# genjax-community/genjax

Hardware: AMD Instinct MI355X
Metric: particle_steps_per_sec (higher is better)
Workload: dtype f32; 1 GPU; gmm_c8_d16 ImportanceK: propagate+reweight+LSE, systematic resample, gather (BASELINE.json configs[1]); k_particles_per_gpu=1048576, k_particles_total=1048576, rng_stream=flat, exchange=none

## Files before the change

### genjax_amd/csrc/gjx_resample.hip

```cpp
#include <math.h>
#include <string.h>

#include "gjx_device.h"
#include "gjx_host.h"
#include "gjx_scan.h"
#include "gjx_tile.h"

namespace gjx {

struct PickPair {
  float v;
  int32_t i;
};

GJX_DEV void pick_better(float& v, int32_t& i, float ov, int32_t oi) {
  if (ov > v || (ov == v && oi < i)) { v = ov; i = oi; }
}

template <int RNG>
__global__ __launch_bounds__(256) void k_pick_partial(const float* logw, int64_t K, int64_t offset, const float* lse,
                                                     key2 key, PickPair* partials) {
  __shared__ float rv[4];
  __shared__ int32_t ri[4];
  const float l = lse[2];
// ... 115 lines not shown
  const int64_t base = (int64_t)blockIdx.x * kScanTile + (int64_t)threadIdx.x * kScanItems;
  uint64_t s = 0;
#pragma unroll
  for (int k = 0; k < kScanItems; ++k)
    if (base + k < K) s += weight_q(x, base + k, is_log, mx);
  s = wave_sum_u64(s);
  if ((threadIdx.x & 63) == 0) red[threadIdx.x >> 6] = s;
  __syncthreads();
  if (threadIdx.x == 0) block_sums[blockIdx.x] = red[0] + red[1] + red[2] + red[3];
}

__global__ __launch_bounds__(256) void k_wscan_write(const float* x, int64_t K, int is_log, const float* lse,
                                                    int n_partials, const uint64_t* block_sums, uint64_t* cum,
                                                    uint64_t* base_total) {
  __shared__ uint64_t wsum[4];
  __shared__ uint64_t red[4];
  __shared__ float fred[8];
  const float mx = block_ref_max(is_log, lse, n_partials, fred, nullptr);
  const int64_t base = (int64_t)blockIdx.x * kScanTile + (int64_t)threadIdx.x * kScanItems;
  uint64_t pre = 0;
  for (int t = threadIdx.x; t < (int)blockIdx.x; t += 256) pre += block_sums[t];
  pre = wave_sum_u64(pre);
  if ((threadIdx.x & 63) == 0) red[threadIdx.x >> 6] = pre;
  uint64_t q[kScanItems];
  uint64_t s = 0;
#pragma unroll
  for (int k = 0; k < kScanItems; ++k) {
    q[k] = (base + k < K) ? weight_q(x, base + k, is_log, mx) : 0;
    s += q[k];
    q[k] = s;
  }
  uint64_t inc = wave_scan_u64(s);
  if ((threadIdx.x & 63) == 63) wsum[threadIdx.x >> 6] = inc;
  __syncthreads();
  uint64_t off = red[0] + red[1] + red[2] + red[3] + inc - s;
  for (int w = 0; w < (int)(threadIdx.x >> 6); ++w) off += wsum[w];
#pragma unroll
  for (int k = 0; k < kScanItems; ++k)
    if (base + k < K) cum[base + k] = off + q[k];
  if (blockIdx.x == gridDim.x - 1 && threadIdx.x == 255) {
    base_total[0] = 0;
    base_total[1] = off + s;
  }
}

GJX_DEV int64_t upper_search(const uint64_t* __restrict__ cum, int64_t K, uint64_t t) {
  int64_t lo = 0, hi = K - 1;
  while (lo < hi) {
    const int64_t mid = (lo + hi) >> 1;
    if (cum[mid] > t) hi = mid; else lo = mid + 1;
  }
  return lo;
}

GJX_DEV int64_t upper_search_in(const uint64_t* __restrict__ cum, int64_t lo, int64_t hi, uint64_t t) {
  while (lo < hi) {
    const int64_t mid = (lo + hi) >> 1;
    if (cum[mid] > t) hi = mid; else lo = mid + 1;
  }
  return lo;
}

template <bool GATHER>
__global__ __launch_bounds__(256) void k_systematic_expand(const uint64_t* __restrict__ cum, int64_t K,
                                                          const uint64_t* base_total, double u, int64_t N_total,
                                                          int64_t out_begin, int64_t n_out, int32_t* ancestors,
                                                          const float* __restrict__ src, int64_t src_stride, int rows,
                                                          float* __restrict__ dst, int64_t dst_stride,
                                                          const int64_t* range_dev = nullptr) {
  constexpr int kOwn = 8;
  if (range_dev) {
    out_begin = range_dev[0];
    const int64_t n = range_dev[1];
    n_out = n < n_out ? n : n_out;
  }
  __shared__ int n_heavy;
  __shared__ int32_t h_i[256];
  __shared__ int64_t h_lo[256], h_hi[256];
  if (threadIdx.x == 0) n_heavy = 0;
  __syncthreads();
  const int64_t i = (int64_t)blockIdx.x * 256 + threadIdx.x;
  const uint64_t base = base_total[0], total = base_total[1];
  const double step = (double)total / (double)N_total;
  const double inv_step = (double)N_total / (double)total;
  const bool in = i < K && total > 0;
  const uint64_t c_cur = in ? base + cum[i] : 0;
  const int64_t j_cur = in ? slots_below(c_cur, u, step, inv_step, total, N_total) : 0;
  int64_t j_prev = __shfl_up((long long)j_cur, 1, 64);
  uint64_t c_prev = __shfl_up((unsigned long long)c_cur, 1, 64);
  if ((threadIdx.x & 63) == 0) {
    c_prev = base + ((in && i > 0) ? cum[i - 1] : 0);
    j_prev = in ? slots_below(c_prev, u, step, inv_step, total, N_total) : 0;
  }
  if (in) {
    if (c_cur > c_prev) {
      int64_t lo = j_prev - out_begin;
      int64_t hi = j_cur - out_begin;
      lo = lo < 0 ? 0 : lo;
      hi = hi > n_out ? n_out : hi;
      if (hi - lo > kOwn) {
        const int h = atomicAdd(&n_heavy, 1);
        h_i[h] = (int32_t)i; h_lo[h] = lo; h_hi[h] = hi;
      } else if (hi > lo) {
        if (ancestors) for (int64_t j = lo; j < hi; ++j) ancestors[j] = (int32_t)i;
        if (GATHER) {
          for (int r = 0; r < rows; ++r) {
            const float v = src[(int64_t)r * src_stride + i];
            for (int64_t j = lo; j < hi; ++j) dst[(int64_t)r * dst_stride + j] = v;
          }
        }
      }
    }
  }
  __syncthreads();
  const int nh = n_heavy;
  for (int h = 0; h < nh; ++h) {
    const int32_t pi = h_i[h];
    const int64_t lo = h_lo[h], hi = h_hi[h];
    if (ancestors) for (int64_t j = lo + threadIdx.x; j < hi; j += 256) ancestors[j] = pi;
    if (GATHER) {
      for (int r = 0; r < rows; ++r) {
        const float v = src[(int64_t)r * src_stride + pi];
        for (int64_t j = lo + threadIdx.x; j < hi; j += 256) dst[(int64_t)r * dst_stride + j] = v;
      }
    }
  }
}

template <int ITEMS>
__global__ __launch_bounds__(256) void k_resample_fused(const float* __restrict__ x, int64_t K, int mode,
                                                       const float* lse, int n_partials, float* lse_out,
                                                       float log_k_total, double u, int64_t N, int32_t* ancestors,
                                                       uint64_t* cum_out, uint64_t* base_total_out,
                                                       unsigned long long* agg, unsigned* ctrl) {
  __shared__ float fred[8];
  __shared__ ScanSmem sm;
  unsigned epoch;
  const unsigned long long tag = grid_tag(ctrl, &epoch);
  const int64_t i0 = ((int64_t)blockIdx.x * 256 + threadIdx.x) * ITEMS;
  float xv[ITEMS];
#pragma unroll
  for (int k = 0; k < ITEMS; ++k) xv[k] = (i0 + k < K) ? x[i0 + k] : 0.0f;
  float sm_sum;
  const float mx = block_ref_max(mode, lse, n_partials, fred, &sm_sum);
  if (mode == 2 && lse_out && blockIdx.x == 0 && threadIdx.x == 0) {
    const float l = mx > -INFINITY ? mx + logf(sm_sum) : -INFINITY;
    lse_out[0] = mx; lse_out[1] = sm_sum; lse_out[2] = l; lse_out[3] = l - log_k_total;
  }
  tile_scan_expand<ITEMS, false>(xv, mode, mx, i0, K, u, N, ancestors, cum_out, base_total_out, agg, tag, ctrl, epoch, true, sm);
}

constexpr int kGatherMaxTiles = 1024;

template <int ITEMS>
__global__ __launch_bounds__(256) void k_resample_gather(const float* __restrict__ x, int64_t K, int mode,
                                                        const float* lse, int n_partials, float* lse_out,
                                                        float log_k_total, double u, const float* __restrict__ src,
                                                        int64_t src_stride, int rows, float* __restrict__ dst,
                                                        int64_t dst_stride, int32_t* ancestors,
                                                        unsigned long long* agg, unsigned* ctrl,
                                                        unsigned long long* timeline) {
#define GJX_STAMP(n) do { if (timeline && threadIdx.x == 0) timeline[blockIdx.x * 8 + (n)] = __builtin_amdgcn_s_memrealtime(); } while (0)
  GJX_STAMP(0);
  constexpr int TILE = 256 * ITEMS;
  __shared__ float fred[8];
  __shared__ uint64_t wsum[4];
  __shared__ uint64_t P[kGatherMaxTiles + 1];
  constexpr int CH = 3;
  __shared__ uint64_t cumL[CH * TILE];
  __shared__ uint64_t s_wtot[CH][4];
  __shared__ int s_range[2];
  unsigned epoch;
  const unsigned long long tag = grid_tag(ctrl, &epoch);
  const int nb = (int)gridDim.x;
  const int lane = threadIdx.x & 63, wid = threadIdx.x >> 6;
  const int64_t i0 = ((int64_t)blockIdx.x * 256 + threadIdx.x) * ITEMS;
  auto load_tile = [&](int64_t p0, float (&v)[ITEMS]) {
    if (ITEMS == 4 && p0 + 4 <= K) {
      const float4 q4 = *(const float4*)(x + p0);
      v[0] = q4.x; v[1] = q4.y; v[2] = q4.z; v[3] = q4.w;
    } else {
#pragma unroll
      for (int k = 0; k < ITEMS; ++k) v[k] = (p0 + k < K) ? x[p0 + k] : 0.0f;
    }
  };
  const int w0 = (int)blockIdx.x - 1;
  float xv[ITEMS], xn[2][ITEMS];
  load_tile(i0, xv);
  float sm_sum;
  const float mx = block_ref_max(mode, lse, n_partials, fred, &sm_sum);
  if (mode == 2 && lse_out && blockIdx.x == 0 && threadIdx.x == 0) {
    const float l = mx > -INFINITY ? mx + logf(sm_sum) : -INFINITY;
    lse_out[0] = mx; lse_out[1] = sm_sum; lse_out[2] = l; lse_out[3] = l - log_k_total;
  }
  uint64_t qown[ITEMS], sown = 0, incown;
  {
#pragma unroll
    for (int k = 0; k < ITEMS; ++k) { sown += (i0 + k < K) ? weight_q(xv, k, mode, mx) : 0; qown[k] = sown; }
    incown = wave_scan_u64(sown);
    if (lane == 63) { wsum[wid] = incown; s_wtot[1][wid] = incown; }
    __syncthreads();
    if (threadIdx.x == 0) grid_publish(agg, tag, wsum[0] + wsum[1] + wsum[2] + wsum[3]);
  }
  GJX_STAMP(1);
#pragma unroll
  for (int c = 0; c < 2; ++c) {
    const int tc = w0 + 2 * c;
#pragma unroll
    for (int k = 0; k < ITEMS; ++k) xn[c][k] = 0.0f;
    if (tc >= 0 && tc < nb) load_tile((int64_t)tc * TILE + (int64_t)threadIdx.x * ITEMS, xn[c]);
  }
  {
    uint64_t qn[2][ITEMS], sn[2], incn[2];
#pragma unroll
    for (int c = 0; c < 2; ++c) {
      const int tc = w0 + 2 * c;
      const bool on = tc >= 0 && tc < nb;
      const int64_t p0 = (int64_t)tc * TILE + (int64_t)threadIdx.x * ITEMS;
      sn[c] = 0;
#pragma unroll
      for (int k = 0; k < ITEMS; ++k) { sn[c] += (on && p0 + k < K) ? weight_q(xn[c], k, mode, mx) : 0; qn[c][k] = sn[c]; }
    }
#pragma unroll
    for (int c = 0; c < 2; ++c) incn[c] = wave_scan_u64(sn[c]);
    if (lane == 63) { s_wtot[0][wid] = incn[0]; s_wtot[2][wid] = incn[1]; }
    __syncthreads();
#pragma unroll
    for (int c = 0; c < 3; ++c) {
      uint64_t base = c == 1 ? incown - sown : incn[c >> 1] - sn[c >> 1];
      for (int w = 0; w < wid; ++w) base += s_wtot[c][w];
#pragma unroll
      for (int k = 0; k < ITEMS; ++k) cumL[c * TILE + threadIdx.x * ITEMS + k] = base + (c == 1 ? qown[k] : qn[c >> 1][k]);
    }
  }
  grid_gather(agg, tag, ctrl, [&](int b, unsigned long long val) { P[b + 1] = val; });
  if (threadIdx.x == 0) P[0] = 0;
  __syncthreads();
  GJX_STAMP(2);
  {
    const int per = (nb + 255) >> 8;
    const int e0 = threadIdx.x * per, e1 = (e0 + per) < nb ? (e0 + per) : nb;
    uint64_t loc = 0;
    for (int e = e0; e < e1; ++e) loc += P[e + 1];
    uint64_t inc = wave_scan_u64(loc);
    if (lane == 63) wsum[wid] = inc;
    __syncthreads();
    uint64_t run = inc - loc;
    for (int w = 0; w < wid; ++w) run += wsum[w];
    for (int e = e0; e < e1; ++e) { run += P[e + 1]; P[e + 1] = run; }
    __syncthreads();
  }
  const uint64_t total = P[nb];
  GJX_STAMP(6);
  if (blockIdx.x == 0 && threadIdx.x == 0) {
    __hip_atomic_store(&ctrl[0], epoch + 1u, __ATOMIC_RELAXED, __HIP_MEMORY_SCOPE_AGENT);
    if (total == 0) __hip_atomic_fetch_or(&ctrl[2], kStatusZeroTotal, __ATOMIC_RELAXED, __HIP_MEMORY_SCOPE_AGENT);
  }
  int32_t anc[ITEMS];
#pragma unroll
  for (int k = 0; k < ITEMS; ++k) anc[k] = (int32_t)((i0 + k < K) ? i0 + k : 0);
  if (total > 0) {
    const double step = (double)total / (double)K;
    uint64_t T[ITEMS];
    int tile[ITEMS], kpos[ITEMS];
#pragma unroll
    for (int k = 0; k < ITEMS; ++k) {
      const int64_t j = (i0 + k < K) ? i0 + k : K - 1;
      T[k] = comb_threshold(j, u, step, total);
      tile[k] = 0;
    }
    auto descend = [&](int k0, int k1) {
#pragma unroll
      for (int sft = kGatherMaxTiles >> 1; sft >= 1; sft >>= 1) {
        const int pa = tile[k0] + sft, pb = tile[k1] + sft;
        if (pa <= nb - 1 && P[pa] <= T[k0]) tile[k0] = pa;
        if (k1 != k0 && pb <= nb - 1 && P[pb] <= T[k1]) tile[k1] = pb;
      }
    };
    const int wlo = (int)blockIdx.x - 4 < 0 ? 0 : ((int)blockIdx.x - 4 > nb - 8 ? (nb - 8 < 0 ? 0 : nb - 8) : (int)blockIdx.x - 4);
    uint64_t Pw[9];
#pragma unroll
    for (int k = 0; k < 9; ++k) Pw[k] = P[wlo + k < nb ? wlo + k : nb];
    if (T[0] >= Pw[0] && T[ITEMS - 1] < Pw[8]) {
#pragma unroll
      for (int k = 0; k < ITEMS; ++k) {
        int tl = wlo;
#pragma unroll
        for (int w = 1; w < 8; ++w) tl += Pw[w] <= T[k] ? 1 : 0;
        tile[k] = tl;
      }
    } else {
      descend(0, ITEMS - 1);
      if (ITEMS > 2) {
        if (tile[0] == tile[ITEMS - 1]) {
#pragma unroll
          for (int k = 1; k < ITEMS - 1; ++k) tile[k] = tile[0];
        } else {
          descend(1, ITEMS > 3 ? 2 : 1);
        }
      }
    }
    if (timeline) { asm volatile("" :: "v"(tile[0]), "v"(tile[ITEMS - 1])); GJX_STAMP(7); }
    if (threadIdx.x == 0) s_range[0] = tile[0];
    if (threadIdx.x == 255) s_range[1] = tile[ITEMS - 1];
    __syncthreads();
    const int tmin = s_range[0], ntiles = s_range[1] - tmin + 1;
    if (tmin >= w0 && s_range[1] <= w0 + 2) {
      GJX_STAMP(3);
      int pos[ITEMS];
      const uint64_t* cm[ITEMS];
      uint64_t Tr[ITEMS];
#pragma unroll
      for (int k = 0; k < ITEMS; ++k) { cm[k] = cumL + (tile[k] - w0) * TILE; Tr[k] = T[k] - P[tile[k]]; pos[k] = 0; }
#pragma unroll
      for (int q = TILE >> 2; q >= 1; q >>= 2) {
#pragma unroll
        for (int k = 0; k < ITEMS; ++k) {
          const uint64_t pa = cm[k][pos[k] + q - 1], pb = cm[k][pos[k] + 2 * q - 1], pc = cm[k][pos[k] + 3 * q - 1];
          pos[k] += (pa <= Tr[k] ? q : 0) + (pb <= Tr[k] ? q : 0) + (pc <= Tr[k] ? q : 0);
        }
      }
#pragma unroll
      for (int k = 0; k < ITEMS; ++k) anc[k] = (int32_t)((int64_t)tile[k] * TILE + pos[k]);
    } else {
#pragma unroll
    for (int k = 0; k < ITEMS; ++k) kpos[k] = tile[k] - tmin;
    auto next_live = [&](int at) { while (at < ntiles && P[tmin + at + 1] == P[tmin + at]) ++at; return at; };
    GJX_STAMP(3);
    float nv[CH][ITEMS];
#pragma unroll
    for (int c = 0; c < CH; ++c)
      if (c < ntiles) load_tile((int64_t)(tmin + c) * TILE + (int64_t)threadIdx.x * ITEMS, nv[c]);
    for (int idx = 0; idx < ntiles;) {
      const int nidx = next_live(idx + CH);
      uint64_t qi[CH][ITEMS], sacc[CH], inc[CH];
      int tsrc[CH];
#pragma unroll
      for (int c = 0; c < CH; ++c) {
        const bool on = idx + c < ntiles;
        tsrc[c] = on ? tmin + idx + c : 0;
        const int64_t p0 = (int64_t)tsrc[c] * TILE + (int64_t)threadIdx.x * ITEMS;
        sacc[c] = 0;
#pragma unroll
        for (int k = 0; k < ITEMS; ++k) { sacc[c] += (on && p0 + k < K) ? weight_q(nv[c], k, mode, mx) : 0; qi[c][k] = sacc[c]; }
        if (nidx + c < ntiles) load_tile((int64_t)(tmin + nidx + c) * TILE + (int64_t)threadIdx.x * ITEMS, nv[c]);
        inc[c] = sacc[c];
      }
#pragma unroll
      for (int c = 0; c < CH; ++c) inc[c] = wave_scan_u64(inc[c]);
      if (lane == 63) {
#pragma unroll
        for (int c = 0; c < CH; ++c) s_wtot[c][wid] = inc[c];
      }
      __syncthreads();
#pragma unroll
      for (int c = 0; c < CH; ++c) {
        uint64_t base = P[tsrc[c]] + (inc[c] - sacc[c]);
        for (int w = 0; w < wid; ++w) base += s_wtot[c][w];
#pragma unroll
        for (int k = 0; k < ITEMS; ++k) cumL[c * TILE + threadIdx.x * ITEMS + k] = base + qi[c][k];
      }
      __syncthreads();
      int pos[ITEMS];
      const uint64_t* cm[ITEMS];
      bool mine[ITEMS];
#pragma unroll
      for (int k = 0; k < ITEMS; ++k) {
        mine[k] = kpos[k] >= idx && kpos[k] < idx + CH;
        cm[k] = cumL + (mine[k] ? (kpos[k] - idx) * TILE : 0);
        pos[k] = 0;
      }
#pragma unroll
      for (int q = TILE >> 2; q >= 1; q >>= 2) {
#pragma unroll
        for (int k = 0; k < ITEMS; ++k) {
          const uint64_t pa = cm[k][pos[k] + q - 1], pb = cm[k][pos[k] + 2 * q - 1], pc = cm[k][pos[k] + 3 * q - 1];
          pos[k] += (pa <= T[k] ? q : 0) + (pb <= T[k] ? q : 0) + (pc <= T[k] ? q : 0);
        }
      }
#pragma unroll
      for (int k = 0; k < ITEMS; ++k)
        if (mine[k]) anc[k] = (int32_t)((int64_t)tile[k] * TILE + pos[k]);
      idx = nidx;
    }
    }
  }
  GJX_STAMP(4);
#pragma unroll
  for (int k = 0; k < ITEMS; ++k) anc[k] = max(0, min(anc[k], (int32_t)(K - 1)));
  const bool whole = i0 + ITEMS <= K;
  if (ancestors) {
    if (ITEMS == 4 && whole) *(int4*)(ancestors + i0) = make_int4(anc[0], anc[1], anc[2], anc[3]);
    else {
#pragma unroll
      for (int k = 0; k < ITEMS; ++k) if (i0 + k < K) ancestors[i0 + k] = anc[k];
    }
  }
  const bool vec = ITEMS == 4 && whole && (dst_stride & 3) == 0 && (((uintptr_t)dst) & 15) == 0;
  if (vec) {
#pragma unroll 4
    for (int r = 0; r < rows; ++r) {
      const float* sr = src + (int64_t)r * src_stride;
      float4 v;
      v.x = sr[anc[0]]; v.y = sr[anc[ITEMS > 1 ? 1 : 0]]; v.z = sr[anc[ITEMS > 2 ? 2 : 0]]; v.w = sr[anc[ITEMS > 3 ? 3 : 0]];
      *(float4*)(dst + (int64_t)r * dst_stride + i0) = v;
    }
  } else {
#pragma unroll 4
    for (int r = 0; r < rows; ++r) {
      const float* sr = src + (int64_t)r * src_stride;
#pragma unroll
      for (int k = 0; k < ITEMS; ++k) if (i0 + k < K) dst[(int64_t)r * dst_stride + i0 + k] = sr[anc[k]];
    }
  }
  GJX_STAMP(5);
#undef GJX_STAMP
}

constexpr int kGatherTiledMaxTiles = 65536;

template <bool GATED>
__global__ __launch_bounds__(kTileQ) void k_tile_totals(const float* __restrict__ logw, int64_t K, uint64_t* S, int32_t* E, const int32_t* gate) {
  constexpr int NW = kTileQ / 64;
  if (GATED && *gate == 0) return;
  __shared__ float fred[NW];
  __shared__ uint64_t wsum[NW];
  const int lane = threadIdx.x & 63, wid = threadIdx.x >> 6;
  const int64_t i = (int64_t)blockIdx.x * kTileQ + threadIdx.x;
  const float lw = i < K ? logw[i] : -INFINITY;
  const float wm = wave_max(lw);
  if (lane == 0) fred[wid] = wm;
  __syncthreads();
  float bm = fred[0];
#pragma unroll
  for (int w = 1; w < NW; ++w) bm = fmaxf(bm, fred[w]);
  const int e = tile_exponent(bm);
  const uint64_t tot_w = wave_total_u64(i < K ? tile_q(lw, e) : 0);
  if (lane == 0) wsum[wid] = tot_w;
  __syncthreads();
  if (threadIdx.x == 0) {
    uint64_t tot = 0;
    for (int w = 0; w < NW; ++w) tot += wsum[w];
    S[blockIdx.x] = tot;
    E[blockIdx.x] = tot ? e : kTileDead;
  }
}

template <int ITEMS, bool PLANNED, bool GATED>
__global__ __launch_bounds__(256) void k_resample_gather_tiled(const float* __restrict__ x, int64_t K, const uint64_t* __restrict__ S,
                                                              const int32_t* __restrict__ E, const uint64_t* __restrict__ Pg,
                                                              const int32_t* __restrict__ shg, int lse_mode, const float* lse,
                                                              int n_partials, float* lse_out, float log_k_total, double u,
                                                              const float* __restrict__ src, int64_t src_stride, int rows,
                                                              float* __restrict__ dst, int64_t dst_stride, int32_t* ancestors,
                                                              unsigned* ctrl, unsigned long long* timeline, const int32_t* gate) {
#define GJX_STAMP(n) do { if (timeline && threadIdx.x == 0) timeline[blockIdx.x * 8 + (n)] = __builtin_amdgcn_s_memrealtime(); } while (0)
  GJX_STAMP(0);
  static_assert(ITEMS == 4, "a block consumes one quantisation tile: 256 lanes x 4 slots");
  extern __shared__ __align__(16) unsigned char gt_dyn[];
  const int nt = (int)gridDim.x;
  uint64_t* const Pl = (uint64_t*)gt_dyn;
  int32_t* const Ebl = (int32_t*)(Pl + ((nt + 2) & ~1));
  __shared__ TiledSearchShared sh;
  const int64_t i0 = ((int64_t)blockIdx.x * 256 + threadIdx.x) * ITEMS;
  int32_t anc[ITEMS];
  if (GATED && *gate == 0) {
#pragma unroll
    for (int k = 0; k < ITEMS; ++k) anc[k] = (int32_t)((i0 + k < K) ? i0 + k : K - 1);
  } else
  tiled_search_tile<PLANNED>(x, K, S, E, Pg, shg, nt, (int)blockIdx.x, Pl, Ebl, sh, lse_mode, lse, n_partials, lse_out, log_k_total, u, ctrl, timeline, anc);
  GJX_STAMP(4);
  const bool whole = i0 + ITEMS <= K;
  if (ancestors) {
    if (whole) *(int4*)(ancestors + i0) = make_int4(anc[0], anc[1], anc[2], anc[3]);
    else {
#pragma unroll
      for (int k = 0; k < ITEMS; ++k) if (i0 + k < K) ancestors[i0 + k] = anc[k];
    }
  }
  const bool vec = whole && (dst_stride & 3) == 0 && (((uintptr_t)dst) & 15) == 0;
  if (vec) {
// ... 131 lines not shown
  s2 = wave_sum(s2);
  if (lane == 0) { red[4 + wid] = s1; red[8 + wid] = s2; }
  __syncthreads();
  if (threadIdx.x == 0) {
    const float b1 = (red[4] + red[5]) + (red[6] + red[7]), b2 = (red[8] + red[9]) + (red[10] + red[11]);
    __hip_atomic_store(&a.pm[blockIdx.x], pack_f2(bm, b1), __ATOMIC_RELAXED, __HIP_MEMORY_SCOPE_AGENT);
    __hip_atomic_store(&a.p2[blockIdx.x], __float_as_uint(b2), __ATOMIC_RELAXED, __HIP_MEMORY_SCOPE_AGENT);
    asm volatile("s_waitcnt vmcnt(0)" ::: "memory");
    const unsigned t = __hip_atomic_fetch_add(a.ticket, 1u, __ATOMIC_RELAXED, __HIP_MEMORY_SCOPE_AGENT);
    red[12] = (t == (unsigned)(nt - 1)) ? 1.0f : 0.0f;
  }
  __syncthreads();
  if (red[12] == 0.0f) return;
  float M = -INFINITY;
  for (int b = threadIdx.x; b < nt; b += 256)
    M = fmaxf(M, __uint_as_float((unsigned)__hip_atomic_load(&a.pm[b], __ATOMIC_RELAXED, __HIP_MEMORY_SCOPE_AGENT)));
  M = wave_max(M);
  if (lane == 0) fin[wid] = M;
  __syncthreads();
  M = fmaxf(fmaxf(fin[0], fin[1]), fmaxf(fin[2], fin[3]));
  float S1 = 0.0f, S2 = 0.0f;
  if (M > -INFINITY) {
    const int per = (nt + 255) >> 8;
    const int b0 = threadIdx.x * per, b1 = b0 + per < nt ? b0 + per : nt;
    for (int b = b0; b < b1; ++b) {
      const unsigned long long v = __hip_atomic_load(&a.pm[b], __ATOMIC_RELAXED, __HIP_MEMORY_SCOPE_AGENT);
      const float t2 = __uint_as_float(__hip_atomic_load(&a.p2[b], __ATOMIC_RELAXED, __HIP_MEMORY_SCOPE_AGENT));
      const float f = fast_exp(__uint_as_float((unsigned)v) - M);
      S1 = fmaf(__uint_as_float((unsigned)(v >> 32)), f, S1);
      S2 = fmaf(t2, f * f, S2);
    }
  }
  S1 = wave_sum(S1);
  S2 = wave_sum(S2);
  if (lane == 0) { fin[4 + wid] = S1; fin[8 + wid] = S2; }
  __syncthreads();
  if (threadIdx.x == 0) {
    S1 = (fin[4] + fin[5]) + (fin[6] + fin[7]);
    S2 = (fin[8] + fin[9]) + (fin[10] + fin[11]);
    const bool live = M > -INFINITY && S2 > 0.0f;
    const float ess = live ? S1 * S1 / S2 : 0.0f;
    if (!ACC) { a.out4[0] = M; a.out4[1] = S1; a.out4[2] = S2; a.out4[3] = ess; }
    if (ACC) {
      const bool fresh = a.fresh ? *a.fresh != 0 : true;
      const float ls = logf(S1);
      const float l = live ? M + ls : -INFINITY;
      float d = l - a.log_k;
      if (!fresh && a.lse_prev) d = live ? (M - a.lse_prev[0]) + (ls - logf(a.lse_prev[1])) : -INFINITY;
      a.lse_rec[0] = M; a.lse_rec[1] = S1; a.lse_rec[2] = l; a.lse_rec[3] = d;
      a.ess_out[0] = ess;
      if (a.decide_out) a.decide_out[0] = (a.always || ess < a.tau_k) ? 1 : 0;
    }
    __hip_atomic_store(a.ticket, 0u, __ATOMIC_RELAXED, __HIP_MEMORY_SCOPE_AGENT);
  }
}

static int ess_workspace(void* workspace, size_t workspace_bytes, int64_t nt, EssArgs& a) {
  if (!workspace || workspace_bytes < kWsHeaderBytes + 12 * (size_t)nt) return -1;
  a.ticket = (unsigned*)workspace;
  a.pm = (unsigned long long*)((char*)workspace + kWsHeaderBytes);
  a.p2 = (unsigned*)(a.pm + nt);
  return 0;
}

int launch_ess_accumulate(const float* inc, float* W, float* w_copy, int64_t K, const int32_t* fresh, float* lse_rec, const float* lse_prev,
                          float* ess_out, int32_t* decide_out, float tau, void* workspace, size_t workspace_bytes, hipStream_t st) {
  const int64_t nt = (K + kTileQ - 1) / kTileQ;
  EssArgs a;
  memset(&a, 0, sizeof(a));
  if (ess_workspace(workspace, workspace_bytes, nt, a)) return gjx_fail(GJX_EWORKSPACE, "gjx_scan_filter_adaptive: workspace too small");
  a.inc = inc; a.W = W; a.w_copy = w_copy; a.K = K; a.fresh = fresh; a.lse_rec = lse_rec; a.lse_prev = lse_prev;
  a.log_k = (float)log((double)K); a.ess_out = ess_out; a.decide_out = decide_out; a.tau_k = tau * (float)K; a.always = tau >= 1.0f;
  hipLaunchKernelGGL(k_ess_tiles<true>, dim3((unsigned)nt), dim3(256), 0, st, a);
  GJX_CHECK_LAUNCH("gjx_scan_filter_adaptive(weights + ESS)");
  return GJX_OK;
}

}

using namespace gjx;

extern "C" int gjx_categorical_pick(const float* logw, int64_t K, int64_t particle_offset, const float* lse,
                                    uint32_t key0, uint32_t key1, int32_t rng_mode, void* out_dev,
                                    void* workspace, size_t workspace_bytes, void* stream) {
  if (!logw || !lse || !out_dev || K <= 0) return gjx_fail(GJX_EINVAL, "gjx_categorical_pick: bad argument");
  if (!workspace || workspace_bytes < gjx_workspace_bytes(GJX_OP_PICK, K)) return gjx_fail(GJX_EWORKSPACE, "gjx_categorical_pick: workspace too small");
  hipStream_t st = (hipStream_t)stream;
  const int64_t want = (K + 1023) / 1024;
  const int nblocks = (int)(want < 2048 ? (want < 1 ? 1 : want) : 2048);
  PickPair* partials = (PickPair*)((char*)workspace + kWsHeaderBytes);
  if (rng_mode == GJX_RNG_JAX32)
    hipLaunchKernelGGL(k_pick_partial<GJX_RNG_JAX32>, dim3(nblocks), dim3(256), 0, st, logw, K, particle_offset, lse, key2{key0, key1}, partials);
  else
    hipLaunchKernelGGL(k_pick_partial<GJX_RNG_FLAT>, dim3(nblocks), dim3(256), 0, st, logw, K, particle_offset, lse, key2{key0, key1}, partials);
  GJX_CHECK_LAUNCH("gjx_categorical_pick/partial");
  hipLaunchKernelGGL(k_pick_finish, dim3(1), dim3(256), 0, st, (const PickPair*)partials, nblocks, (PickPair*)out_dev);
  GJX_CHECK_LAUNCH("gjx_categorical_pick/finish");
  return GJX_OK;
}

extern "C" int gjx_trials_lse_pick(const float* logw, int64_t n_trials, int64_t K, int64_t particle_offset, uint32_t key0, uint32_t key1,
                                   int32_t rng_mode, float* lse_out, int32_t* pick_out, void* stream) {
  if (!logw || !lse_out || n_trials <= 0 || K <= 0 || n_trials > 0x7fffffffLL || particle_offset < 0 ||
      (pick_out && particle_offset + n_trials * K > 0x7fffffffLL))
    return gjx_fail(GJX_EINVAL, "gjx_trials_lse_pick: bad argument");
  hipStream_t st = (hipStream_t)stream;
  const float log_k = (float)log((double)K);
  if (rng_mode == GJX_RNG_JAX32)
    hipLaunchKernelGGL(k_trials_lse_pick<GJX_RNG_JAX32>, dim3((unsigned)n_trials), dim3(256), 0, st, logw, K, particle_offset, key2{key0, key1},
                       pick_out ? 1 : 0, log_k, lse_out, pick_out);
  else
    hipLaunchKernelGGL(k_trials_lse_pick<GJX_RNG_FLAT>, dim3((unsigned)n_trials), dim3(256), 0, st, logw, K, particle_offset, key2{key0, key1},
                       pick_out ? 1 : 0, log_k, lse_out, pick_out);
  GJX_CHECK_LAUNCH("gjx_trials_lse_pick");
  return GJX_OK;
}

extern "C" int gjx_weight_cumsum(const float* x, int64_t K, int32_t is_log, const float* lse, int32_t n_partials,
                                 uint64_t* cum, uint64_t* base_total_dev, float* lse_out, int64_t K_total,
                                 void* workspace, size_t workspace_bytes, void* stream) {
  if (!x || !cum || !base_total_dev || K <= 0 || is_log < 0 || is_log > 2 || (is_log && !lse) || (is_log == 2 && n_partials <= 0))
    return gjx_fail(GJX_EINVAL, "gjx_weight_cumsum: bad argument");
  if (!workspace || workspace_bytes < gjx_workspace_bytes(GJX_OP_RESAMPLE, K)) return gjx_fail(GJX_EWORKSPACE, "gjx_weight_cumsum: workspace too small");
  hipStream_t st = (hipStream_t)stream;
  const int nblocks = (int)((K + kScanTile - 1) / kScanTile);
  uint64_t* bs = (uint64_t*)((char*)workspace + kWsHeaderBytes);
  const float log_k = (float)log((double)(K_total > 0 ? K_total : K));
  hipLaunchKernelGGL(k_wsum_blocks, dim3(nblocks), dim3(256), 0, st, x, K, (int)is_log, lse, (int)n_partials, lse_out, log_k, bs);
  GJX_CHECK_LAUNCH("gjx_weight_cumsum/sum");
  hipLaunchKernelGGL(k_wscan_write, dim3(nblocks), dim3(256), 0, st, x, K, (int)is_log, lse, (int)n_partials, (const uint64_t*)bs, cum, base_total_dev);
  GJX_CHECK_LAUNCH("gjx_weight_cumsum/write");
  return GJX_OK;
}

extern "C" int gjx_resample_systematic(const uint64_t* cum, int64_t K, const uint64_t* base_total_dev, double u,
                                       int64_t N_total, int64_t out_begin, int64_t n_out, int32_t* ancestors,
                                       void* stream) {
  if (!cum || !base_total_dev || !ancestors || K <= 0 || N_total <= 0 || n_out < 0 || !(u >= 0.0 && u < 1.0))
    return gjx_fail(GJX_EINVAL, "gjx_resample_systematic: bad argument");
  if (n_out == 0) return GJX_OK;
  hipLaunchKernelGGL(k_systematic_expand<false>, dim3((unsigned)((K + 255) / 256)), dim3(256), 0, (hipStream_t)stream, cum, K,
                     base_total_dev, u, N_total, out_begin, n_out, ancestors, (const float*)nullptr, (int64_t)0, 0,
                     (float*)nullptr, (int64_t)0);
  GJX_CHECK_LAUNCH("gjx_resample_systematic");
  return GJX_OK;
}

static int env_items() {
  const char* e = getenv("GJX_RESAMPLE_ITEMS");
  const int v = e ? atoi(e) : 0;
  return (v == 1 || v == 4 || v == 16) ? v : 0;
}

extern "C" int gjx_resample_indices(const float* x, int64_t K, int32_t is_log, const float* lse, int32_t n_partials,
                                    double u, int64_t N, int32_t* ancestors, uint64_t* cum, uint64_t* base_total_dev,
                                    float* lse_out, int64_t K_total, void* workspace, size_t workspace_bytes, void* stream) {
  if (!x || K <= 0 || N <= 0 || is_log < 0 || is_log > 2 || (is_log && !lse) || (is_log == 2 && n_partials <= 0) ||
      !(u >= 0.0 && u < 1.0) || (!ancestors && !cum))
    return gjx_fail(GJX_EINVAL, "gjx_resample_indices: bad argument");
  if (!workspace || workspace_bytes < gjx_workspace_bytes(GJX_OP_RESAMPLE, K)) return gjx_fail(GJX_EWORKSPACE, "gjx_resample_indices: workspace too small");
  int items = env_items();
  int64_t nblocks = 0;
  const int cand[3] = {1, 4, 16};
  bool fits = false;
  for (int c = 0; c < 3 && !fits; ++c) {
    if (items && cand[c] != items) continue;
    const void* fn = cand[c] == 1 ? (const void*)k_resample_fused<1> : cand[c] == 4 ? (const void*)k_resample_fused<4> : (const void*)k_resample_fused<16>;
    const int cap = gjx_coresident_blocks(fn, 256, 0);
    nblocks = (K + 256 * (int64_t)cand[c] - 1) / (256 * (int64_t)cand[c]);
    if (nblocks <= cap) { items = cand[c]; fits = true; }
  }
  hipStream_t st = (hipStream_t)stream;
  if (!fits || !ancestors) {
    if (!cum || !base_total_dev) return gjx_fail(GJX_EUNSUPPORTED, "gjx_resample_indices: the grid would not be co-resident on this device and there are no cum/base_total buffers for the three-launch path");
    int rc = gjx_weight_cumsum(x, K, is_log, lse, n_partials, cum, base_total_dev, lse_out, K_total, workspace, workspace_bytes, stream);
    if (rc || !ancestors) return rc;
    return gjx_resample_systematic(cum, K, base_total_dev, u, N, 0, N, ancestors, stream);
  }
  unsigned* ctrl = (unsigned*)workspace + 8;
  unsigned long long* agg = (unsigned long long*)((char*)workspace + kWsHeaderBytes);
  const float log_k = (float)log((double)(K_total > 0 ? K_total : K));
#define GJX_RF(IT) hipLaunchKernelGGL((k_resample_fused<IT>), dim3((unsigned)nblocks), dim3(256), 0, st, x, K, (int)is_log, lse, \
                                      (int)n_partials, lse_out, log_k, u, N, ancestors, cum, base_total_dev, agg, ctrl)
  if (items == 1) GJX_RF(1); else if (items == 4) GJX_RF(4); else GJX_RF(16);
#undef GJX_RF
  GJX_CHECK_LAUNCH("gjx_resample_indices");
  return GJX_OK;
}

extern "C" int gjx_resample_gather(const float* x, int64_t K, int32_t is_log, const float* lse, int32_t n_partials, double u,
                                   const float* src, int64_t src_stride, int32_t rows, float* dst, int64_t dst_stride,
                                   int32_t* ancestors, float* lse_out, int64_t K_total, void* workspace,
                                   size_t workspace_bytes, void* stream) {
  if (!x || K <= 0 || is_log < 0 || is_log > 2 || (is_log && !lse) || (is_log == 2 && n_partials <= 0) ||
      !(u >= 0.0 && u < 1.0) || rows < 0 || (rows > 0 && (!src || !dst)) || K > 0x7fffffffLL)
    return gjx_fail(GJX_EINVAL, "gjx_resample_gather: bad argument");
  if (!workspace || workspace_bytes < gjx_workspace_bytes(GJX_OP_RESAMPLE, K)) return gjx_fail(GJX_EWORKSPACE, "gjx_resample_gather: workspace too small");
  int items = 0;
  int64_t nblocks = 0;
  const int cand[2] = {1, 4};
  const int forced = env_items();
  for (int c = 0; c < 2 && !items; ++c) {
    if (forced && cand[c] != forced) continue;
    const void* fn = cand[c] == 1 ? (const void*)k_resample_gather<1> : (const void*)k_resample_gather<4>;
    const int cap = gjx_coresident_blocks(fn, 256, 0);
    nblocks = (K + 256 * (int64_t)cand[c] - 1) / (256 * (int64_t)cand[c]);
    if (nblocks <= cap && nblocks <= kGatherMaxTiles) items = cand[c];
  }
  if (!items) return gjx_fail(GJX_EUNSUPPORTED, "gjx_resample_gather: K is too large for one co-resident grid on this device (use gjx_resample_indices + gjx_gather_rows)");
  hipStream_t st = (hipStream_t)stream;
  unsigned* ctrl = (unsigned*)workspace + 8;
  unsigned long long* agg = (unsigned long long*)((char*)workspace + kWsHeaderBytes);
  const float log_k = (float)log((double)(K_total > 0 ? K_total : K));
  unsigned long long* timeline = nullptr;
  timeline = gjx::debug_timeline(64 * (size_t)nblocks);
#define GJX_RG(IT) hipLaunchKernelGGL((k_resample_gather<IT>), dim3((unsigned)nblocks), dim3(256), 0, st, x, K, (int)is_log, lse, \
                                      (int)n_partials, lse_out, log_k, u, src, src_stride, (int)rows, dst, dst_stride, ancestors, agg, ctrl, timeline)
  if (items == 1) GJX_RG(1); else GJX_RG(4);
#undef GJX_RG
  GJX_CHECK_LAUNCH("gjx_resample_gather");
  return GJX_OK;
}

int gjx::resample_gather_tiled_gated(const float* logw, int64_t K, const uint64_t* tile_S, const int32_t* tile_E, int32_t lse_mode,
                                     const float* lse, int32_t n_partials, double u, const float* src, int64_t src_stride,
                                     int32_t rows, float* dst, int64_t dst_stride, int32_t* ancestors, float* lse_out,
                                     int64_t K_total, void* workspace, size_t workspace_bytes, void* stream, const int32_t* gate) {
  if (!logw || K <= 0 || !(u >= 0.0 && u < 1.0) || rows < 0 || (rows > 0 && (!src || !dst)) || K > 0x7fffffffLL ||
      (lse_mode != 0 && lse_mode != 2) || (lse_mode == 2 && (!lse || n_partials <= 0)) || ((tile_S == nullptr) != (tile_E == nullptr)))
    return gjx_fail(GJX_EINVAL, "gjx_resample_gather_tiled: bad argument");
  const int64_t nt = (K + kTileQ - 1) / kTileQ;
  if (nt > kGatherTiledMaxTiles) return gjx_fail(GJX_EUNSUPPORTED, "gjx_resample_gather_tiled: more than 65536 tiles (K > 2^26): use gjx_resample_indices_tiled + gjx_gather_rows");
  if (!workspace || workspace_bytes < gjx_workspace_bytes(GJX_OP_RESAMPLE, K) || kWsHeaderBytes + 12 * (size_t)nt > workspace_bytes)
    return gjx_fail(GJX_EWORKSPACE, "gjx_resample_gather_tiled: workspace too small");
  hipStream_t st = (hipStream_t)stream;
  unsigned* ctrl = (unsigned*)workspace + 8;
  if (!tile_S) {
    uint64_t* S = (uint64_t*)((char*)workspace + kWsHeaderBytes);
    int32_t* E = (int32_t*)(S + nt);
    if (gate) hipLaunchKernelGGL(k_tile_totals<true>, dim3((unsigned)nt), dim3(kTileQ), 0, st, logw, K, S, E, gate);
    else hipLaunchKernelGGL(k_tile_totals<false>, dim3((unsigned)nt), dim3(kTileQ), 0, st, logw, K, S, E, (const int32_t*)nullptr);
    GJX_CHECK_LAUNCH("gjx_resample_gather_tiled/totals");
    tile_S = S; tile_E = E;
  }
  const float log_k = (float)log((double)(K_total > 0 ? K_total : K));
  unsigned long long* timeline = gjx::debug_timeline(64 * (size_t)nt);
  if (nt > 1024 || getenv("GJX_TILED_PLANNED")) {
    uint64_t* Pg = (uint64_t*)((char*)workspace + kWsHeaderBytes + 12 * (size_t)nt + 16);
    Pg = (uint64_t*)(((uintptr_t)Pg + 15) & ~(uintptr_t)15);
    int32_t* shg = (int32_t*)(Pg + nt + 1);
    if ((char*)(shg + nt) > (char*)workspace + workspace_bytes) return gjx_fail(GJX_EWORKSPACE, "gjx_resample_gather_tiled: workspace too small");
    const int rc = gjx::launch_tiled_plan(tile_S, tile_E, (int)nt, Pg, shg, ctrl, st, gate);
    if (rc) return rc;
#define GJX_GT(GATED) hipLaunchKernelGGL((k_resample_gather_tiled<4, true, GATED>), dim3((unsigned)nt), dim3(256), 0, st, logw, K, tile_S, tile_E, \
                       (const uint64_t*)Pg, (const int32_t*)shg, (int)lse_mode, lse, (int)n_partials, lse_out, log_k, u, src, src_stride, (int)rows, \
                       dst, dst_stride, ancestors, ctrl, timeline, gate)
    if (gate) GJX_GT(true); else GJX_GT(false);
#undef GJX_GT
  } else {
    const size_t lds = 8 * (size_t)((nt + 2) & ~1) + 4 * (size_t)nt;
#define GJX_GT(GATED) hipLaunchKernelGGL((k_resample_gather_tiled<4, false, GATED>), dim3((unsigned)nt), dim3(256), lds, st, logw, K, tile_S, tile_E, \
                       (const uint64_t*)nullptr, (const int32_t*)nullptr, (int)lse_mode, lse, (int)n_partials, lse_out, log_k, u, src, src_stride, \
                       (int)rows, dst, dst_stride, ancestors, ctrl, timeline, gate)
    if (gate) GJX_GT(true); else GJX_GT(false);
#undef GJX_GT
  }
  GJX_CHECK_LAUNCH("gjx_resample_gather_tiled");
  return GJX_OK;
}

extern "C" int gjx_resample_gather_tiled(const float* logw, int64_t K, const uint64_t* tile_S, const int32_t* tile_E, int32_t lse_mode,
                                         const float* lse, int32_t n_partials, double u, const float* src, int64_t src_stride,
                                         int32_t rows, float* dst, int64_t dst_stride, int32_t* ancestors, float* lse_out,
                                         int64_t K_total, void* workspace, size_t workspace_bytes, void* stream) {
  return gjx::resample_gather_tiled_gated(logw, K, tile_S, tile_E, lse_mode, lse, n_partials, u, src, src_stride, rows, dst, dst_stride, ancestors,
                                          lse_out, K_total, workspace, workspace_bytes, stream, nullptr);
}

extern "C" int gjx_resample_gather_systematic(const uint64_t* cum, int64_t K, const uint64_t* base_total_dev, double u,
                                              int64_t N_total, int64_t out_begin, int64_t n_out, const float* src,
                                              int64_t src_stride, int32_t rows, float* dst, int64_t dst_stride,
                                              int32_t* ancestors, void* stream) {
  if (!cum || !base_total_dev || !src || !dst || !ancestors || K <= 0 || N_total <= 0 || n_out < 0 || rows < 0 ||
      !(u >= 0.0 && u < 1.0))
    return gjx_fail(GJX_EINVAL, "gjx_resample_gather_systematic: bad argument");
  if (n_out == 0) return GJX_OK;
  const int rc = gjx_resample_systematic(cum, K, base_total_dev, u, N_total, out_begin, n_out, ancestors, stream);
  if (rc) return rc;
  return gjx_gather_rows(src, src_stride, ancestors, n_out, rows, dst, dst_stride, stream);
}

extern "C" int gjx_resample_multinomial(const uint64_t* cum, int64_t K, const uint64_t* base_total_dev,
                                        uint32_t key0, uint32_t key1, int64_t N_total, int64_t out_begin,
                                        int64_t n_out, int32_t* ancestors, void* stream) {
  (void)N_total;
  if (!cum || !base_total_dev || !ancestors || K <= 0 || n_out < 0) return gjx_fail(GJX_EINVAL, "gjx_resample_multinomial: bad argument");
  if (n_out == 0) return GJX_OK;
  hipLaunchKernelGGL(k_multinomial, dim3((unsigned)((n_out + 255) / 256)), dim3(256), 0, (hipStream_t)stream, cum, K,
                     base_total_dev, key2{key0, key1}, out_begin, n_out, ancestors);
  GJX_CHECK_LAUNCH("gjx_resample_multinomial");
  return GJX_OK;
}

extern "C" int gjx_gather_rows(const float* src, int64_t src_stride, const int32_t* anc, int64_t n_out, int32_t rows,
                               float* dst, int64_t dst_stride, void* stream) {
  if (!src || !anc || !dst || n_out < 0 || rows < 0) return gjx_fail(GJX_EINVAL, "gjx_gather_rows: bad argument");
  if (n_out == 0 || rows == 0) return GJX_OK;
  hipLaunchKernelGGL(k_gather_rows, dim3((unsigned)((n_out + 255) / 256)), dim3(256), 0, (hipStream_t)stream, src,
                     src_stride, anc, n_out, (int)rows, dst, dst_stride);
  GJX_CHECK_LAUNCH("gjx_gather_rows");
  return GJX_OK;
}


extern "C" int gjx_ess(const float* logw, int64_t K, float* out4, void* workspace, size_t workspace_bytes, void* stream) {
  if (!logw || !out4 || K <= 0 || K > (int64_t)1 << 31) return gjx_fail(GJX_EINVAL, "gjx_ess: bad argument");
  const int64_t nt = (K + kTileQ - 1) / kTileQ;
  EssArgs a;
  memset(&a, 0, sizeof(a));
  if (workspace_bytes < gjx_workspace_bytes(GJX_OP_RESAMPLE, K) || ess_workspace(workspace, workspace_bytes, nt, a))
    return gjx_fail(GJX_EWORKSPACE, "gjx_ess: workspace too small");
  a.W = const_cast<float*>(logw); a.K = K; a.out4 = out4;
  hipLaunchKernelGGL(k_ess_tiles<false>, dim3((unsigned)nt), dim3(256), 0, (hipStream_t)stream, a);
  GJX_CHECK_LAUNCH("gjx_ess");
  return GJX_OK;
}
```

### profiles/microbench/gather_timeline.py

```python
import os, sys, torch, numpy as np
sys.path.insert(0, os.path.dirname(os.path.dirname(os.path.dirname(os.path.abspath(__file__)))))
from genjax_amd import kernels, workloads, _abi as A
K = 1 << 20
prog, _ = workloads.gmm_program()
ws = kernels.workspace(A.OP_RUN, K, "cuda"); ws2 = kernels.workspace(A.OP_RESAMPLE, K, "cuda")
out = kernels.run_program(prog, (0, 1), K, ws=ws, want_weight=False, want_lse=False)
n_part = kernels.run_partials_count(prog, K, 0)
rows = torch.empty_like(out["choices"]); lse = torch.empty(4, device="cuda")
def go():
    kernels.run_program(prog, (0, 2), K, ws=ws, out=out, want_weight=False, want_lse=False)
    kernels.resample_gather(out["logw"], 0.37, out["choices"], partials=(ws, n_part), lse_out=lse, out=rows, ws=ws2, allow_fallback=False)
for _ in range(20): go()
tl = torch.zeros((1024, 8), dtype=torch.int64, device="cuda")
from genjax_amd._lib import load as _load
import ctypes as _C
_load().gjx_debug_timeline(_C.c_void_p(tl.data_ptr()), tl.numel() * tl.element_size())
go(); torch.cuda.synchronize()
t = tl.cpu().numpy().astype(np.float64); t0 = t[:, 0].min()
for j, n in [(0, "start"), (1, "tile total published"), (2, "totals gathered"), (6, "prefix of totals"), (7, "source tiles found"), (3, "tile list known"), (4, "ancestors known"), (5, "rows copied (end)")]:
    c = (t[:, j] - t0) * 0.01
    print(f"{n:24s} min {c.min():7.2f}  median {np.median(c):7.2f}  max {c.max():7.2f} us")
```

Before: 18.63 billion particle-steps/s.

## Add push-form resample-gather where each block emits slots owned by its tile

Adds a 'push' path to the fused resample-gather kernel. Each block reduces the gathered tile totals to get its own prefix and the grand total, works out which systematic-resample slots fall inside its own tile's weight range, and binary-searches its local cumulative weights to write those ancestors and rows. This skips loading the neighbouring tiles, the block-wide prefix scan over all tile totals, and the search across tiles. It falls back to the old slot form when one tile's weight is too concentrated (more than 2*TILE slots) or when GJX_RESAMPLE_FORM=slot. In exchange, blocks can get uneven amounts of work, and writes go to output slots outside the block's own index range.

```diff
diff --git a/genjax_amd/csrc/gjx_resample.hip b/genjax_amd/csrc/gjx_resample.hip
--- a/genjax_amd/csrc/gjx_resample.hip
+++ b/genjax_amd/csrc/gjx_resample.hip
@@ -291,6 +291,90 @@
 
 constexpr int kGatherMaxTiles = 1024;
 
+template <unsigned CTRL, unsigned ROW_MASK>
+GJX_DEV uint64_t dpp_max_u64(uint64_t v) {
+  const uint32_t lo = dpp_mov<CTRL, ROW_MASK>(0u, (uint32_t)v), hi = dpp_mov<CTRL, ROW_MASK>(0u, (uint32_t)(v >> 32));
+  const uint64_t o = ((uint64_t)hi << 32) | lo;
+  return o > v ? o : v;
+}
+GJX_DEV uint64_t wave_scan_max_u64(uint64_t v) {
+  v = dpp_max_u64<kDppShr1, 0xf>(v);
+  v = dpp_max_u64<kDppShr2, 0xf>(v);
+  v = dpp_max_u64<kDppShr4, 0xf>(v);
+  v = dpp_max_u64<kDppShr8, 0xf>(v);
+  v = dpp_max_u64<kDppBcast15, 0xa>(v);
+  v = dpp_max_u64<kDppBcast31, 0xc>(v);
+  return v;
+}
+
+template <int ITEMS, int NG>
+GJX_DEV void push_groups(const uint64_t* cum, int64_t jb0, int64_t run_lo, int64_t run_hi, int64_t K, double u, double step,
+                         uint64_t total, uint64_t Pb, int64_t tile_base, const float* __restrict__ src, int64_t src_stride,
+                         int rows, float* __restrict__ dst, int64_t dst_stride, int32_t* ancestors, bool vec_ok,
+                         unsigned long long* stamp) {
+  constexpr int TILE = 256 * ITEMS;
+  bool ok[NG][ITEMS];
+  uint64_t Tr[NG][ITEMS];
+  int pos[NG][ITEMS];
+#pragma unroll
+  for (int g = 0; g < NG; ++g)
+#pragma unroll
+    for (int k = 0; k < ITEMS; ++k) {
+      const int64_t j = jb0 + (int64_t)g * TILE + k;
+      ok[g][k] = j >= run_lo && j < run_hi;
+      Tr[g][k] = comb_threshold(ok[g][k] ? j : run_lo, u, step, total) - Pb;
+      pos[g][k] = 0;
+    }
+#pragma unroll
+  for (int q = TILE >> 2; q >= 1; q >>= 2) {
+#pragma unroll
+    for (int g = 0; g < NG; ++g)
+#pragma unroll
+      for (int k = 0; k < ITEMS; ++k) {
+        const uint64_t pa = cum[pos[g][k] + q - 1], pb = cum[pos[g][k] + 2 * q - 1], pc = cum[pos[g][k] + 3 * q - 1];
+        pos[g][k] += (pa <= Tr[g][k] ? q : 0) + (pb <= Tr[g][k] ? q : 0) + (pc <= Tr[g][k] ? q : 0);
+      }
+  }
+  int32_t anc[NG][ITEMS];
+#pragma unroll
+  for (int g = 0; g < NG; ++g)
+#pragma unroll
+    for (int k = 0; k < ITEMS; ++k) anc[g][k] = max(0, min((int32_t)(tile_base + pos[g][k]), (int32_t)(K - 1)));
+  if (stamp) { asm volatile("" :: "v"(anc[0][0])); *stamp = __builtin_amdgcn_s_memrealtime(); }
+  bool all[NG];
+#pragma unroll
+  for (int g = 0; g < NG; ++g) all[g] = ok[g][0] && ok[g][ITEMS - 1];
+  if (ancestors) {
+#pragma unroll
+    for (int g = 0; g < NG; ++g) {
+      int32_t* a = ancestors + jb0 + (int64_t)g * TILE;
+      if (ITEMS == 4 && all[g]) *(int4*)a = make_int4(anc[g][0], anc[g][ITEMS > 1 ? 1 : 0], anc[g][ITEMS > 2 ? 2 : 0], anc[g][ITEMS > 3 ? 3 : 0]);
+      else {
+#pragma unroll
+        for (int k = 0; k < ITEMS; ++k) if (ok[g][k]) a[k] = anc[g][k];
+      }
+    }
+  }
+#pragma unroll 4
+  for (int r = 0; r < rows; ++r) {
+    const float* sr = src + (int64_t)r * src_stride;
+    float v[NG][ITEMS];
+#pragma unroll
+    for (int g = 0; g < NG; ++g)
+#pragma unroll
+      for (int k = 0; k < ITEMS; ++k) v[g][k] = ok[g][k] ? sr[anc[g][k]] : 0.0f;
+#pragma unroll
+    for (int g = 0; g < NG; ++g) {
+      float* d = dst + (int64_t)r * dst_stride + jb0 + (int64_t)g * TILE;
+      if (ITEMS == 4 && vec_ok && all[g]) *(float4*)d = make_float4(v[g][0], v[g][ITEMS > 1 ? 1 : 0], v[g][ITEMS > 2 ? 2 : 0], v[g][ITEMS > 3 ? 3 : 0]);
+      else {
+#pragma unroll
+        for (int k = 0; k < ITEMS; ++k) if (ok[g][k]) d[k] = v[g][k];
+      }
+    }
+  }
+}
+
 template <int ITEMS>
 __global__ __launch_bounds__(256) void k_resample_gather(const float* __restrict__ x, int64_t K, int mode,
                                                         const float* lse, int n_partials, float* lse_out,
@@ -298,16 +382,19 @@
                                                         int64_t src_stride, int rows, float* __restrict__ dst,
                                                         int64_t dst_stride, int32_t* ancestors,
                                                         unsigned long long* agg, unsigned* ctrl,
-                                                        unsigned long long* timeline) {
+                                                        unsigned long long* timeline, int force_slot) {
 #define GJX_STAMP(n) do { if (timeline && threadIdx.x == 0) timeline[blockIdx.x * 8 + (n)] = __builtin_amdgcn_s_memrealtime(); } while (0)
   GJX_STAMP(0);
   constexpr int TILE = 256 * ITEMS;
+  constexpr int kPushCap = 2 * TILE;
   __shared__ float fred[8];
   __shared__ uint64_t wsum[4];
   __shared__ uint64_t P[kGatherMaxTiles + 1];
   constexpr int CH = 3;
   __shared__ uint64_t cumL[CH * TILE];
   __shared__ uint64_t s_wtot[CH][4];
+  __shared__ uint64_t s_red[3][4];
+  __shared__ int64_t s_run[2];
   __shared__ int s_range[2];
   unsigned epoch;
   const unsigned long long tag = grid_tag(ctrl, &epoch);
@@ -342,6 +429,59 @@
     if (threadIdx.x == 0) grid_publish(agg, tag, wsum[0] + wsum[1] + wsum[2] + wsum[3]);
   }
   GJX_STAMP(1);
+  {
+    uint64_t base = incown - sown;
+    for (int w = 0; w < wid; ++w) base += s_wtot[1][w];
+#pragma unroll
+    for (int k = 0; k < ITEMS; ++k) cumL[TILE + threadIdx.x * ITEMS + k] = base + qown[k];
+  }
+  uint64_t g_pre = 0, g_tot = 0, g_big = 0;
+  grid_gather(agg, tag, ctrl, [&](int b, unsigned long long val) {
+    P[b + 1] = val;
+    g_tot += val;
+    if (b < (int)blockIdx.x) g_pre += val;
+    g_big = val > g_big ? val : g_big;
+  });
+  if (threadIdx.x == 0) P[0] = 0;
+  g_pre = wave_scan_u64(g_pre);
+  g_tot = wave_scan_u64(g_tot);
+  g_big = wave_scan_max_u64(g_big);
+  if (lane == 63) { s_red[0][wid] = g_pre; s_red[1][wid] = g_tot; s_red[2][wid] = g_big; }
+  __syncthreads();
+  const uint64_t Pb = s_red[0][0] + s_red[0][1] + s_red[0][2] + s_red[0][3];
+  const uint64_t total = s_red[1][0] + s_red[1][1] + s_red[1][2] + s_red[1][3];
+  uint64_t big = s_red[2][0];
+#pragma unroll
+  for (int w = 1; w < 4; ++w) big = s_red[2][w] > big ? s_red[2][w] : big;
+  GJX_STAMP(2);
+  if (blockIdx.x == 0 && threadIdx.x == 0) {
+    __hip_atomic_store(&ctrl[0], epoch + 1u, __ATOMIC_RELAXED, __HIP_MEMORY_SCOPE_AGENT);
+    if (total == 0) __hip_atomic_fetch_or(&ctrl[2], kStatusZeroTotal, __ATOMIC_RELAXED, __HIP_MEMORY_SCOPE_AGENT);
+  }
+  if (!force_slot && total > 0 && (double)big * (double)K <= (double)total * (double)(kPushCap - 2)) {
+    const double step = (double)total / (double)K, inv_step = (double)K / (double)total;
+    const uint64_t Sb = s_wtot[1][0] + s_wtot[1][1] + s_wtot[1][2] + s_wtot[1][3];
+    if (threadIdx.x == 0) s_run[0] = slots_below(Pb, u, step, inv_step, total, K);
+    if (threadIdx.x == 64) s_run[1] = slots_below(Pb + Sb, u, step, inv_step, total, K);
+    __syncthreads();
+    int64_t run_lo = s_run[0], run_hi = s_run[1];
+    run_lo = run_lo < 0 ? 0 : (run_lo > K ? K : run_lo);
+    run_hi = run_hi > K ? K : run_hi;
+    run_hi = run_hi > run_lo + kPushCap ? run_lo + kPushCap : run_hi;
+    GJX_STAMP(3);
+    const int64_t g0 = run_lo & ~(int64_t)(ITEMS - 1);
+    const bool vec_ok = (dst_stride & 3) == 0 && (((uintptr_t)dst) & 15) == 0;
+    unsigned long long* stamp = (timeline && threadIdx.x == 0) ? &timeline[blockIdx.x * 8 + 4] : nullptr;
+    for (int64_t jw = g0 + (int64_t)wid * 64 * ITEMS; jw < run_hi; jw += 2 * TILE) {
+      const int64_t jb = jw + (int64_t)lane * ITEMS;
+      if (jw + TILE < run_hi)
+        push_groups<ITEMS, 2>(cumL + TILE, jb, run_lo, run_hi, K, u, step, total, Pb, (int64_t)blockIdx.x * TILE, src, src_stride, rows, dst, dst_stride, ancestors, vec_ok, stamp);
+      else
+        push_groups<ITEMS, 1>(cumL + TILE, jb, run_lo, run_hi, K, u, step, total, Pb, (int64_t)blockIdx.x * TILE, src, src_stride, rows, dst, dst_stride, ancestors, vec_ok, stamp);
+    }
+    GJX_STAMP(5);
+    return;
+  }
 #pragma unroll
   for (int c = 0; c < 2; ++c) {
     const int tc = w0 + 2 * c;
@@ -365,17 +505,13 @@
     if (lane == 63) { s_wtot[0][wid] = incn[0]; s_wtot[2][wid] = incn[1]; }
     __syncthreads();
 #pragma unroll
-    for (int c = 0; c < 3; ++c) {
-      uint64_t base = c == 1 ? incown - sown : incn[c >> 1] - sn[c >> 1];
+    for (int c = 0; c < 3; c += 2) {
+      uint64_t base = incn[c >> 1] - sn[c >> 1];
       for (int w = 0; w < wid; ++w) base += s_wtot[c][w];
 #pragma unroll
-      for (int k = 0; k < ITEMS; ++k) cumL[c * TILE + threadIdx.x * ITEMS + k] = base + (c == 1 ? qown[k] : qn[c >> 1][k]);
-    }
-  }
-  grid_gather(agg, tag, ctrl, [&](int b, unsigned long long val) { P[b + 1] = val; });
-  if (threadIdx.x == 0) P[0] = 0;
-  __syncthreads();
-  GJX_STAMP(2);
+      for (int k = 0; k < ITEMS; ++k) cumL[c * TILE + threadIdx.x * ITEMS + k] = base + qn[c >> 1][k];
+    }
+  }
   {
     const int per = (nb + 255) >> 8;
     const int e0 = threadIdx.x * per, e1 = (e0 + per) < nb ? (e0 + per) : nb;
@@ -389,12 +525,7 @@
     for (int e = e0; e < e1; ++e) { run += P[e + 1]; P[e + 1] = run; }
     __syncthreads();
   }
-  const uint64_t total = P[nb];
   GJX_STAMP(6);
-  if (blockIdx.x == 0 && threadIdx.x == 0) {
-    __hip_atomic_store(&ctrl[0], epoch + 1u, __ATOMIC_RELAXED, __HIP_MEMORY_SCOPE_AGENT);
-    if (total == 0) __hip_atomic_fetch_or(&ctrl[2], kStatusZeroTotal, __ATOMIC_RELAXED, __HIP_MEMORY_SCOPE_AGENT);
-  }
   int32_t anc[ITEMS];
 #pragma unroll
   for (int k = 0; k < ITEMS; ++k) anc[k] = (int32_t)((i0 + k < K) ? i0 + k : 0);
@@ -445,7 +576,6 @@
     __syncthreads();
     const int tmin = s_range[0], ntiles = s_range[1] - tmin + 1;
     if (tmin >= w0 && s_range[1] <= w0 + 2) {
-      GJX_STAMP(3);
       int pos[ITEMS];
       const uint64_t* cm[ITEMS];
       uint64_t Tr[ITEMS];
@@ -465,7 +595,6 @@
 #pragma unroll
     for (int k = 0; k < ITEMS; ++k) kpos[k] = tile[k] - tmin;
     auto next_live = [&](int at) { while (at < ntiles && P[tmin + at + 1] == P[tmin + at]) ++at; return at; };
-    GJX_STAMP(3);
     float nv[CH][ITEMS];
 #pragma unroll
     for (int c = 0; c < CH; ++c)
@@ -903,6 +1032,11 @@
   return (v == 1 || v == 4 || v == 16) ? v : 0;
 }
 
+static int env_force_slot() {
+  const char* e = getenv("GJX_RESAMPLE_FORM");
+  return (e && !strcmp(e, "slot")) ? 1 : 0;
+}
+
 extern "C" int gjx_resample_indices(const float* x, int64_t K, int32_t is_log, const float* lse, int32_t n_partials,
                                     double u, int64_t N, int32_t* ancestors, uint64_t* cum, uint64_t* base_total_dev,
                                     float* lse_out, int64_t K_total, void* workspace, size_t workspace_bytes, void* stream) {
@@ -966,7 +1100,8 @@
   unsigned long long* timeline = nullptr;
   timeline = gjx::debug_timeline(64 * (size_t)nblocks);
 #define GJX_RG(IT) hipLaunchKernelGGL((k_resample_gather<IT>), dim3((unsigned)nblocks), dim3(256), 0, st, x, K, (int)is_log, lse, \
-                                      (int)n_partials, lse_out, log_k, u, src, src_stride, (int)rows, dst, dst_stride, ancestors, agg, ctrl, timeline)
+                                      (int)n_partials, lse_out, log_k, u, src, src_stride, (int)rows, dst, dst_stride, ancestors, agg, ctrl, timeline, force_slot)
+  const int force_slot = env_force_slot();
   if (items == 1) GJX_RG(1); else GJX_RG(4);
 #undef GJX_RG
   GJX_CHECK_LAUNCH("gjx_resample_gather");
diff --git a/profiles/microbench/gather_timeline.py b/profiles/microbench/gather_timeline.py
--- a/profiles/microbench/gather_timeline.py
+++ b/profiles/microbench/gather_timeline.py
@@ -17,6 +17,11 @@
 _load().gjx_debug_timeline(_C.c_void_p(tl.data_ptr()), tl.numel() * tl.element_size())
 go(); torch.cuda.synchronize()
 t = tl.cpu().numpy().astype(np.float64); t0 = t[:, 0].min()
-for j, n in [(0, "start"), (1, "tile total published"), (2, "totals gathered"), (6, "prefix of totals"), (7, "source tiles found"), (3, "tile list known"), (4, "ancestors known"), (5, "rows copied (end)")]:
-    c = (t[:, j] - t0) * 0.01
-    print(f"{n:24s} min {c.min():7.2f}  median {np.median(c):7.2f}  max {c.max():7.2f} us")
+push = bool((t[:, 3] != 0).all())
+print("form:", "push (blocks write the slots their own tile owns)" if push else "slot (blocks consume the slots [1024 b, 1024 (b + 1)))")
+phases = ([(0, "start"), (1, "tile total published"), (2, "totals gathered + reduced"), (3, "run bounds known"), (4, "ancestors known"), (5, "rows copied (end)")]
+          if push else
+          [(0, "start"), (1, "tile total published"), (2, "totals gathered + reduced"), (6, "window + prefix of totals"), (7, "source tiles found"), (4, "ancestors known"), (5, "rows copied (end)")])
+for j, n in phases:
+    c = (t[:, j][t[:, j] != 0] - t0) * 0.01
+    print(f"{n:28s} min {c.min():7.2f}  median {np.median(c):7.2f}  max {c.max():7.2f} us")
```

New measurement: 16.93 billion particle-steps/s. -9.2%, worse.
